# liuli33/CMLPL

Hardware: AMD Instinct MI355X
Metric: HSI patches/sec per training step (higher is better)
Workload: dtype f32 (convolutions: f32 operands as 3 exact bf16 pieces on the bf16 MFMA, 6 of 9 piece products, f32 accumulate, per-product worst case 2^-21 -- conv1's tap loops of the per-sample kernels as 2 fp16 pieces with power-of-two operand scales, 3 piece products, worst case 2^-20 / mean 2^-23, falling back; 1 GPU; B2: synthetic PaviaU-shaped patches 11x11x103, spectrum 103, 9 classes, 128 labelled + 128 unlabelled rows per GPU (batch 256), dual BaseNet2 fwd/bwd + contrastive/mutual losses + bank + Adam, epoch 1 (memory-bank smoothing active), in-kernel PCG4D noise / Philox dropout; global_batch=256, parallelism=dp1

## Files before the change

### cmlpl_amd/csrc/api.hip

```cpp
#include <hip/hip_runtime.h>
#include <stdlib.h>
#include <string.h>

#include <vector>

#include "../../include/cmlpl.h"
#include "kernels.hpp"

using namespace cmlpl;

namespace {

inline int64_t up4(int64_t v) { return (v + 3) & ~(int64_t)3; }
inline size_t up256(size_t v) { return (v + 255) & ~(size_t)255; }

struct Dims {
  int C, H, W, bands, K, HW, H2, W2, P2, H4, W4, P4, SF, F;
};

bool make_dims(const cmlpl_shape* s, Dims* d) {
  if (!s) return false;
  d->C = s->C; d->H = s->H; d->W = s->W; d->bands = s->bands; d->K = s->K;
  if (d->C < 1 || d->C > 256 || d->H < 4 || d->W < 4 || d->bands < 1 || d->K < 1 || d->K > 64) return false;
  d->HW = d->H * d->W; d->H2 = d->H / 2; d->W2 = d->W / 2; d->P2 = d->H2 * d->W2;
// ... 204 lines not shown
  x.sigma = sigma; x.nlab = b->bt; x.philox = b->noise8 == nullptr;
  x.lab0 = sh ? sh->lab0 : 0; x.unl_base = sh ? sh->bt_g + sh->unl0 : b->bt;
  x.seed = seed; x.step = step;
  return x;
}
int fwd_core(const Dims& d, const NetRoute& r, const cmlpl_layout_t& L, int nets, int n, const float* d_params, int64_t param_stride,
             const float* d_packed, const XSrc& xs, const XSrc* xspec, float* d_sn_out, const long long* d_labels, float* d_labels_f, const float* d_xn,
             const float* d_sn, const float* d_snT,
             const float* d_dropmask, float dropout_p, int train, uint64_t seed, uint64_t step,
             const cmlpl_shard* shard, float* d_logits, float* d_feat, const NetWs& w, hipStream_t st,
             float* xn_save = nullptr, int parts = 3, bool early_feat = false);
int bwd_core(const Dims& d, const NetRoute& r, const cmlpl_layout_t& L, int nets, int n, const float* d_params, int64_t param_stride,
             const float* d_packed, const XSrc& xs, const float* d_xn, const float* d_sn, const float* d_dropmask,
             float dropout_p, int train, const float* d_dlogits, const float* d_dfeat, float* d_grads,
             int64_t grad_stride, const NetWs& w, hipStream_t st, int* dyn_cursor = nullptr, cmlpl_dyn* dyn_table = nullptr,
             int parts = 3);
}

int cmlpl_basenet2_fwd(const cmlpl_shape* shape, int nets, int n, const float* d_params, int64_t param_stride,
                       const float* d_packed, const float* d_xn, const float* d_sn, const float* d_snT,
                       const float* d_dropmask, float dropout_p, int train, uint64_t seed, uint64_t step,
                       const cmlpl_shard* shard,
                       float* d_logits, float* d_feat, void* d_workspace, size_t workspace_bytes, void* stream) {
  Dims d;
  cmlpl_layout_t L;
  if (!make_dims(shape, &d) || cmlpl_layout(shape, &L)) return CMLPL_E_SHAPE;
  if (nets < 1 || nets > 2 || n < 1 || !d_params || !d_packed || !d_xn || !d_sn || !d_logits || !d_feat ||
      !d_workspace)
    return CMLPL_E_ARG;
  if (dropout_p < 0.f || dropout_p >= 1.f) return CMLPL_E_ARG;
  NetRoute r;
// ... 81 lines not shown
  if (nets < 1 || nets > 2 || n < 1 || !d_params || !d_packed || !d_xn || !d_sn || !d_dlogits || !d_grads ||
      !d_workspace)
    return CMLPL_E_ARG;
  NetRoute r;
  NetWs w;
  if (!make_route(d, nets, n, &r) || !carve_net(d, r, nets, n, (char*)d_workspace, &w)) return CMLPL_E_SHAPE;
  if (w.bytes > workspace_bytes) return CMLPL_E_WORKSPACE;
  return bwd_core(d, r, L, nets, n, d_params, param_stride, d_packed,
                  xsrc_plain(d_xn, nets, n, (long long)d.C * d.HW, 0, 0, nullptr), d_xn, d_sn, d_dropmask, dropout_p, train, d_dlogits, d_dfeat, d_grads, grad_stride, w, (hipStream_t)stream);
}

namespace {
int bwd_core(const Dims& d, const NetRoute& r, const cmlpl_layout_t& L, int nets, int n, const float* d_params, int64_t param_stride,
             const float* d_packed, const XSrc& xs, const float* d_xn, const float* d_sn, const float* d_dropmask,
             float dropout_p, int train, const float* d_dlogits, const float* d_dfeat, float* d_grads,
             int64_t grad_stride, const NetWs& w, hipStream_t st, int* dyn_cursor, cmlpl_dyn* dyn_table, int parts) {
  const float* mask = (!train || dropout_p <= 0.f) ? nullptr : (d_dropmask ? d_dropmask : w.dropgen);
  int rc;
  const bool fused_head = r.bwd == ROUTE_A;
  uint32_t* const hstat = r.stats ? w.hstat : nullptr;
  const float* d_dfeat_head = (parts == 3) ? d_dfeat : nullptr;
  GemmTN gw_cls, gw_spe;
  {
    GemmTN& g = gw_cls;
    g.bias_in = nullptr; g.bias_in_bstride = 0; g.relu = 0;
    g.A = d_dlogits; g.a_bstride = (long long)n * d.K; g.lda = d.K; g.M = d.K;
    g.B = w.catd; g.b_bstride = (long long)n * d.F; g.ldb = d.F; g.N = d.F;
    g.C = d_grads + L.param_off[8]; g.c_bstride = grad_stride; g.ldc = d.F;
    g.bias = d_grads + L.param_off[9]; g.bias_bstride = grad_stride;
    g.R = n; g.batches = nets; g.scale = 1.f;
    GemmTN& h = gw_spe;
// ... 43 lines not shown
    if ((rc = TIMED(CMLPL_K_CONV1_WGRAD, chk(launch_wgrad3_pair(nets, n, d.H, d.W, w.a0, w.dp1, w.m1, w.part1, d.H2, d.W2,
                                  w.p1, w.dp2, w.m2, w.part2, &merged, st, hstat, h2flag,
                                  L.packed_total))))) return rc;
    (void)merged;
  }
  if (!(parts & 2)) return 0;
  if (parts == 2) {
    if (!d_dfeat) return CMLPL_E_ARG;
    if ((rc = TIMED(CMLPL_K_HEAD_BWD, chk(launch_dy_fixup(nets, n, w.y, w.ynorm, d_dfeat, w.dy, st))))) return rc;
  }
  ReduceTable rt;
  rt.count = 0; rt.total_blocks = 0; rt.grad_ns = grad_stride; rt.dyn_cursor = dyn_cursor; rt.dyn_table = dyn_table;
  Wgrad3Plan wp1, wp2;
  bool wpair = false;
  if (!plan_wgrad3_both(nets, n, d.H, d.W, d.H2, d.W2, true, &wp1, &wp2, &wpair)) return CMLPL_E_SHAPE;
  reduce_table_add(rt, w.part1, wp1.G, PART3, 1, 64, d_grads + L.param_off[2], d_grads + L.param_off[3]);
  reduce_table_add(rt, w.part2, wp2.G, PART3, 1, 64, d_grads + L.param_off[4], d_grads + L.param_off[5]);
  reduce_table_add(rt, w.part0, conv0_partials(d, r, n), conv0_partial_size(d.C), 0, d.C,
                   d_grads + L.param_off[0], d_grads + L.param_off[1]);
  return TIMED(CMLPL_K_CONV1_WRED, chk(launch_reduce_gemm(nets, rt, gw_cls, gw_spe, st)));
}

int check_batch(const Dims& d, const cmlpl_batch* b) {
  if (!b || b->bt < 1 || b->btu < 1 || !b->d_xl || !b->d_xu) return CMLPL_E_ARG;
  if (b->d_cube == nullptr) return (b->d_xpl && b->d_xpu) ? 0 : CMLPL_E_ARG;
  if (b->d_xpl || b->d_xpu || !b->d_lab_pix || !b->d_unl_pix || b->cube_rows < 1 || b->cube_cols < 1) return CMLPL_E_ARG;
  if (d.H != d.W || b->cube_rows < d.H || b->cube_cols < d.W || cube_feed_lds(d.C, d.W) > LDS_MAX) return CMLPL_E_SHAPE;
  return 0;
}
}

}
namespace {
int forward_impl(const cmlpl_shape* shape, const cmlpl_hparams* hp, const cmlpl_batch* batch, const cmlpl_shard* shard,
                 const float* d_params, const float* d_packed, const float* d_dropmask, int train, uint64_t seed,
// ... 71 lines not shown
  return forward_impl(shape, hp, batch, shard, d_params, d_packed, d_dropmask, train, seed, step, d_logits, nullptr, nullptr,
                      d_workspace, workspace_bytes, stream, DynRef(), 2);
}
int cmlpl_forward(const cmlpl_shape* shape, const cmlpl_hparams* hp, const cmlpl_batch* batch, const cmlpl_shard* shard,
                  const float* d_params, const float* d_packed, const float* d_dropmask, int train, uint64_t seed,
                  uint64_t step, float* d_logits, float* d_feat, float* d_labels_f, void* d_workspace,
                  size_t workspace_bytes, void* stream) {
  return forward_impl(shape, hp, batch, shard, d_params, d_packed, d_dropmask, train, seed, step, d_logits, d_feat,
                      d_labels_f, d_workspace, workspace_bytes, stream, DynRef());
}
}
namespace {
int backward_impl(const cmlpl_shape* shape, const cmlpl_hparams* hp, const cmlpl_batch* batch, const cmlpl_shard* shard,
                  const float* d_params, const float* d_packed, const float* d_dropmask, int train, uint64_t seed,
                  uint64_t step, const float* d_dlogits, const float* d_dfeat, float* d_grads, int64_t grad_stride,
                  void* d_workspace, size_t workspace_bytes, void* stream, DynRef dyn, int* dyn_cursor, int parts = 3);
}
extern "C" {

int cmlpl_backward_data(const cmlpl_shape* shape, const cmlpl_hparams* hp, const cmlpl_batch* batch, const cmlpl_shard* shard,
                        const float* d_params, const float* d_packed, const float* d_dropmask, int train, uint64_t seed,
                        uint64_t step, const float* d_dlogits, void* d_workspace, size_t workspace_bytes, void* stream) {
  return backward_impl(shape, hp, batch, shard, d_params, d_packed, d_dropmask, train, seed, step, d_dlogits, nullptr,
                       nullptr, 0, d_workspace, workspace_bytes, stream, DynRef(), nullptr, 1);
}
int cmlpl_backward_weights(const cmlpl_shape* shape, const cmlpl_hparams* hp, const cmlpl_batch* batch,
                           const cmlpl_shard* shard, const float* d_params, const float* d_packed, const float* d_dropmask,
                           int train, uint64_t seed, uint64_t step, const float* d_dlogits, const float* d_dfeat,
                           float* d_grads, int64_t grad_stride, void* d_workspace, size_t workspace_bytes, void* stream) {
  return backward_impl(shape, hp, batch, shard, d_params, d_packed, d_dropmask, train, seed, step, d_dlogits, d_dfeat,
                       d_grads, grad_stride, d_workspace, workspace_bytes, stream, DynRef(), nullptr, 2);
}

int cmlpl_backward(const cmlpl_shape* shape, const cmlpl_hparams* hp, const cmlpl_batch* batch, const cmlpl_shard* shard,
                   const float* d_params, const float* d_packed, const float* d_dropmask, int train, uint64_t seed,
                   uint64_t step, const float* d_dlogits, const float* d_dfeat, float* d_grads, int64_t grad_stride,
                   void* d_workspace, size_t workspace_bytes, void* stream) {
  return backward_impl(shape, hp, batch, shard, d_params, d_packed, d_dropmask, train, seed, step, d_dlogits, d_dfeat,
                       d_grads, grad_stride, d_workspace, workspace_bytes, stream, DynRef(), nullptr);
}
}
namespace {
int backward_impl(const cmlpl_shape* shape, const cmlpl_hparams* hp, const cmlpl_batch* batch, const cmlpl_shard* shard,
                  const float* d_params, const float* d_packed, const float* d_dropmask, int train, uint64_t seed,
                  uint64_t step, const float* d_dlogits, const float* d_dfeat, float* d_grads, int64_t grad_stride,
                  void* d_workspace, size_t workspace_bytes, void* stream, DynRef dyn, int* dyn_cursor, int parts) {
  Dims d;
  cmlpl_layout_t L;
  if (!make_dims(shape, &d) || cmlpl_layout(shape, &L)) return CMLPL_E_SHAPE;
  if (!hp || !d_params || !d_packed || !d_dlogits || ((parts & 2) && !d_grads) || !d_workspace)
    return CMLPL_E_ARG;
  if (int brc = check_batch(d, batch)) return brc;
  const int n = batch->bt + batch->btu;
  NetRoute r;
  NetWs nw;
  if (!make_route(d, 2, n, &r) || !carve_net(d, r, 2, n, (char*)d_workspace, &nw)) return CMLPL_E_SHAPE;
  StepWs sw;
  carve_step(d, n, n, (char*)d_workspace + nw.bytes, &sw);
  if (nw.bytes + ((char*)sw.dlogits - ((char*)d_workspace + nw.bytes)) > workspace_bytes) return CMLPL_E_WORKSPACE;
  const bool copy = r.xn_copy();
  const XSrc xs = xsrc_plain(sw.xn, 2, n, (long long)d.C * d.HW, seed, step, shard, dyn);
  return bwd_core(d, r, L, 2, n, d_params, L.param_total, d_packed, xs,
                  copy ? sw.xn : nullptr, sw.sn, d_dropmask, hp->dropout_p, train, d_dlogits, d_dfeat, d_grads,
                  grad_stride, nw, (hipStream_t)stream, dyn_cursor, dyn_cursor ? (cmlpl_dyn*)dyn.table : nullptr, parts);
}
}
extern "C" {

namespace {
int fill_loss_args(const Dims& d, const cmlpl_shard* sh, const float* d_logits, const float* d_feat,
                   const int64_t* d_labels, const cmlpl_banks* banks, int smooth, float adap_mask,
                   const cmlpl_hparams* hp, void* ws, size_t ws_bytes, LossArgs* out,
                   const cmlpl_gathered* gth = nullptr, const RowSel* sel = nullptr) {
  if (!sh || !banks || !hp || !ws) return CMLPL_E_ARG;
  if (gth == nullptr && (!d_logits || !d_feat || !d_labels)) return CMLPL_E_ARG;
  if (gth != nullptr && (!gth->d_recv_feat || !gth->d_logits_local || gth->world < 1 || gth->bt_local < 1 || gth->btu_local < 1 ||
                         gth->world * gth->bt_local != sh->bt_g || gth->world * gth->btu_local != sh->btu_g ||
                         sh->nunl != gth->btu_local || sh->unl0 % gth->btu_local != 0 ||
                         (sh->nlab != 0 && (sh->nlab != gth->bt_local || sh->lab0 % gth->bt_local != 0))))
// ... 314 lines not shown
                             io->d_unl_pix};
  if ((rc = forward_impl(shape, hp, &batch, &sh, io->d_params, io->d_packed, io->d_dropmask, train, io->seed,
                         io->step, io->d_logits, io->d_feat, nullptr, io->d_workspace, io->workspace_bytes, stream, dyn, 3,
                         sym_mode)))
    return rc;
  const RowSel sel = batch_sel(&batch, dyn);
  if (cps) {
    if ((rc = cps_loss_impl(shape, io->bt, io->btu, io->d_logits, io->d_labels, hp, io->d_scalars, sw.dlogits,
                            (int64_t*)sw.probs, sw.loss,
                            loss_ws_floats(n, n, n, d.K, io->banks.Q > n ? io->banks.Q : n) * 4, stream, &sel)))
      return rc;
  } else if ((rc = loss_both(shape, io->bt, io->btu, io->d_logits, io->d_feat, io->d_labels, &io->banks,
                      io->smooth, io->adap_mask, hp, io->d_scalars, sw.dlogits, sw.dfeat, sw.probs, sw.loss,
                      loss_ws_floats(n, n, n, d.K, io->banks.Q > n ? io->banks.Q : n) * 4, stream, &sel)))
    return rc;
  if ((rc = backward_impl(shape, hp, &batch, &sh, io->d_params, io->d_packed, io->d_dropmask, train, io->seed,
                          io->step, sw.dlogits, cps ? nullptr : sw.dfeat, io->d_grads, L.param_total, io->d_workspace,
                          io->workspace_bytes, stream, dyn, io->d_dyn_cursor))) return rc;
  if (io->apply_update)
    return adam_impl(shape, 2, io->d_params, L.param_total, io->d_grads, L.param_total, io->d_m, io->d_v,
                     (dyn.table != nullptr && io->adam_t < 1) ? 1 : io->adam_t, hp, io->d_packed, stream, dyn, opt);
  if (opt != nullptr && opt->d_norms != nullptr)
    return grad_norm_impl(shape, 2, io->d_grads, L.param_total, opt->max_norm, opt->d_partials, opt->d_norms, stream, dyn);
  return 0;
}
int cmlpl_train_step(const cmlpl_shape* shape, const cmlpl_hparams* hp, const cmlpl_step_io* io, void* stream) {
  return cmlpl_train_step_opt(shape, hp, io, nullptr, stream);
}

struct StepGraph { hipGraph_t graph; hipGraphExec_t exec; };

int cmlpl_step_graph_create_opt(const cmlpl_shape* shape, const cmlpl_hparams* hp, const cmlpl_step_io* io,
                                const cmlpl_optim* opt, void* stream, void** graph_out) {
// ... 555 lines not shown
```

### cmlpl_amd/csrc/conv0.hip

```cpp
#include "common.hpp"
#include "kernels.hpp"
#include "gemm_tn.hpp"

namespace cmlpl {

constexpr int C0_KMAX = 128;

template <int KCAP>
__global__ __launch_bounds__(256) void conv0_fwd_kernel(const float* __restrict__ xn, const float* __restrict__ w0t,
                                                        long long w0t_ns, const float* __restrict__ b,
                                                        long long pstride, float* __restrict__ a0, int n, int C,
                                                        int HW) {
  extern __shared__ __attribute__((aligned(16))) float wl[];
  const int tid = threadIdx.x, lane = tid & 63, l31 = lane & 31, hh = lane >> 5;
  const int wave = __builtin_amdgcn_readfirstlane(tid >> 6);
  const int net = blockIdx.y;
  const int Cp = (C + 1) & ~1, KK = Cp >> 1;
  const long long M = (long long)n * HW;
  const long long m = ((long long)blockIdx.x * 4 + wave) * 32 + l31;
  const long long mm = (m < M) ? m : 0;
  const int sample = (int)(mm / HW), pix = (int)(mm - (long long)sample * HW);
  const float* ap = xn + ((long long)net * n + sample) * C * HW + pix;
  float av[KCAP];
#pragma unroll
// ... 341 lines not shown
  }
}

__global__ __launch_bounds__(256) void partial_reduce_kernel(ReduceTable t) {
  __shared__ __attribute__((aligned(16))) float red[16][64];
  partial_reduce_block(t, (int)blockIdx.x, (int)blockIdx.y, red);
}

__global__ __launch_bounds__(256) void reduce_gemm_kernel(ReduceTable t, int reduce_blocks, GemmTN2 g) {
  __shared__ GemmTNShared sh;
  const int bid = (int)blockIdx.x;
  if (bid < reduce_blocks) partial_reduce_block(t, bid % t.total_blocks, bid / t.total_blocks, (float (*)[64])&sh.red[0][0][0]);
  else gemm_tn_block(g, bid - reduce_blocks, sh);
}

hipError_t launch_reduce_gemm(int nets, const ReduceTable& t, const GemmTN& g0, const GemmTN& g1, hipStream_t st) {
  GemmTN2 g;
  g.p[0] = g0; g.p[1] = g1; g.nblk0 = gemm_tn_blocks(g0);
  const int rb = t.total_blocks * nets, gb = g.nblk0 + gemm_tn_blocks(g1);
  hipLaunchKernelGGL(reduce_gemm_kernel, dim3(rb + gb), dim3(256), 0, st, t, rb, g);
  return hipGetLastError();
}

void reduce_table_add(ReduceTable& t, const float* part, int G, int PS, int mode, int C, float* dW, float* db) {
  ReduceProb& p = t.p[t.count++];
  p.part = part; p.dW = dW; p.db = db; p.G = G; p.PS = PS; p.mode = mode; p.C = C; p.blk0 = t.total_blocks;
  p.el = 256;
  t.total_blocks += (PS + 255) / 256;
}

hipError_t launch_partial_reduce(int nets, const ReduceTable& t, hipStream_t st) {
  hipLaunchKernelGGL(partial_reduce_kernel, dim3(t.total_blocks, nets), dim3(256), 0, st, t);
  return hipGetLastError();
}

int conv0_partial_size(int C) { return conv0_partial_rows(C) * 64 + 64; }

int plan_conv0_wgrad_G(int n, int C, int HW) {
  (void)C; (void)HW;
  int G = n < 256 ? n : 256;
  return G < 1 ? 1 : G;
}

// ... 27 lines not shown
```

### cmlpl_amd/csrc/gemm_tn.hpp

```cpp
#pragma once
#include "common.hpp"
#include "kernels.hpp"

namespace cmlpl {

constexpr int GT_DEPTH = 16;

struct GemmTN2 { GemmTN p[2]; int nblk0; };
struct GemmTNShared { __attribute__((aligned(16))) float red[3][16][64]; float ared[4][64]; };

__device__ __forceinline__ void gemm_tn_block(const GemmTN2& t, int bid, GemmTNShared& sh) {
  const int tid = threadIdx.x, lane = tid & 63, l31 = lane & 31, hh = lane >> 5;
  const int wave = __builtin_amdgcn_readfirstlane(tid >> 6);
  const int pi = (bid >= t.nblk0) ? 1 : 0;
  const GemmTN g = t.p[pi];
  int b = bid - (pi ? t.nblk0 : 0);
  const int NTg = (g.N + 31) >> 5, MTg = (g.M + 31) >> 5;
  const int nt = b % NTg; b /= NTg;
  const int mt = b % MTg;
  const int bz = b / MTg;
  const float* A = g.A + (long long)bz * g.a_bstride;
  const float* B = g.B + (long long)bz * g.b_bstride;
  const int i = mt * 32 + l31, j = nt * 32 + l31;
  const bool iv = i < g.M, jv = j < g.N;
  const float* ap = A + (iv ? i : 0);
  const float* bp = B + (jv ? j : 0);
  const int R = g.R;
  const int pairs = (R + 1) >> 1;
  const int ppw = (pairs + 3) >> 2;
  const int t0 = wave * ppw, t1 = (t0 + ppw < pairs) ? t0 + ppw : pairs;
  f32x16 acc = zero16();
  float asum = 0.f;
  for (int tb = t0; tb < t1; tb += GT_DEPTH) {
    float av[GT_DEPTH], bv[GT_DEPTH];
    int seg = 0, off = 0;
    if (g.b_seg_rows > 0) { const int r0 = 2 * tb + hh; seg = r0 / g.b_seg_rows; off = r0 - seg * g.b_seg_rows; }
#pragma unroll
    for (int q = 0; q < GT_DEPTH; ++q) {
      const int r = 2 * (tb + q) + hh;
      const bool rv = (tb + q < t1) && (r < R);
      const int rc = rv ? r : 0;
      const long long bo = g.b_seg_rows > 0 ? (rv ? (long long)seg * g.b_seg_stride + (long long)off * g.ldb : 0)
                                            : (long long)rc * g.ldb;
      const float a = ap[(long long)rc * g.lda], b = bp[bo];
      av[q] = (rv && iv) ? a : 0.f;
      bv[q] = (rv && jv) ? b : 0.f;
      off += 2;
      while (g.b_seg_rows > 0 && off >= g.b_seg_rows) { off -= g.b_seg_rows; ++seg; }
    }
#pragma unroll
    for (int q = 0; q < GT_DEPTH; ++q) {
      asum += av[q];
      acc = mfma32(av[q], bv[q], acc);
    }
  }
  if (wave > 0) {
#pragma unroll
    for (int r = 0; r < 16; ++r) sh.red[wave - 1][r][lane] = acc[r];
  }
  sh.ared[wave][lane] = asum;
  __syncthreads();
  if (wave == 0) {
    float* C = g.C + (long long)bz * g.c_bstride;
    if (jv) {
#pragma unroll
      for (int r = 0; r < 16; ++r) {
        const int row = mt * 32 + acc_row(r, lane);
        float v = (((acc[r] + sh.red[0][r][lane]) + sh.red[1][r][lane]) + sh.red[2][r][lane]) * g.scale;
        if (g.bias_in != nullptr) v += g.bias_in[(long long)bz * g.bias_in_bstride + j];
        if (g.relu) v = relu_nan(v);
        if (row < g.M) C[(long long)row * g.ldc + j] = v;
      }
    }
    if (g.bias != nullptr && nt == 0) {
      float tot = (sh.ared[0][lane] + sh.ared[1][lane]) + (sh.ared[2][lane] + sh.ared[3][lane]);
      tot += __shfl_xor(tot, 32, 64);
// ... 9 lines not shown
```

### cmlpl_amd/csrc/kernels.hpp

```cpp
#pragma once
#include <hip/hip_runtime.h>
#include <stdint.h>
#include <stddef.h>
#include <stdlib.h>
#include <atomic>

#include "common.hpp"

namespace cmlpl {

constexpr int PACK_CONV = 9 * 64 * 64;
constexpr int PACK_B3 = PACK_CONV * 3 / 2;
constexpr int PACK_PER_NET = 4 * PACK_B3 + PACK_CONV;
__host__ __device__ inline long long pack_off_b3(int , int , int which) { return (long long)which * PACK_B3; }
__host__ __device__ inline long long pack_off_frag() { return 4LL * PACK_B3; }
__host__ __device__ inline int conv_b3_index(int tap, int k, int n, int p) {
  return ((((tap * 4 + (k >> 4)) * 3 + p) * 2 + (n >> 5)) * 64 + ((k >> 3) & 1) * 32 + (n & 31)) * 8 + (k & 7);
}
__host__ __device__ inline long long pack_off_w0t() { return PACK_PER_NET; }
__host__ __device__ inline long long pack_off_wst(int C) { return PACK_PER_NET + (long long)((C + 1) & ~1) * 64; }
__host__ __device__ inline long long pack_off_w0b3(int C, int bands) { return pack_off_wst(C) + (long long)bands * 1024; }
__host__ __device__ inline long long pack_off_w0b3_end(int C, int bands) { return pack_off_w0b3(C, bands) + (long long)((C + 15) / 16) * 1536; }
constexpr int H2_WEXP = 13;
constexpr int PACK_H2 = PACK_CONV;
// ... 101 lines not shown
hipError_t launch_wgrad3_pair(int nets, int n, int H1, int W1, const float* in1, const float* dpool1,
                              const uint8_t* mask1, float* part1, int H2, int W2, const float* in2,
                              const float* dpool2, const uint8_t* mask2, float* part2, bool* merged, hipStream_t st,
                              const uint32_t* hstat = nullptr ,
                              const uint32_t* h2flag = nullptr, long long h2flag_ns = 0);

hipError_t launch_conv0_fwd(int nets, int n, int C, int HW, const float* xn, const float* w0t, long long w0t_ns,
                            const float* b, long long pstride, float* a0, hipStream_t st);
bool conv0a_ok(int C, int HW);
hipError_t launch_conv0a_fwd(int nets, int n, int C, int HW, const XSrc& xs, const float* w0b3, long long w0b3_ns,
                             const float* b, long long pstride, float* a0, float* xn, hipStream_t st);
int plan_conv0_wgrad_G(int n, int C, int HW);
struct ReduceProb { const float* part; float* dW; float* db; int G, PS, mode, C, blk0, el; };
struct ReduceTable { ReduceProb p[3]; int count, total_blocks; long long grad_ns;
                     int* dyn_cursor; cmlpl_dyn* dyn_table;  };
void reduce_table_add(ReduceTable& t, const float* part, int G, int PS, int mode, int C, float* dW, float* db);
hipError_t launch_partial_reduce(int nets, const ReduceTable& t, hipStream_t st);
struct GemmTN;
hipError_t launch_reduce_gemm(int nets, const ReduceTable& t, const GemmTN& g0, const GemmTN& g1, hipStream_t st);
__host__ __device__ inline int conv0_partial_rows(int C) { return (C + 3) & ~3; }
int conv0_partial_size(int C);
hipError_t launch_conv0_wgrad(int nets, int n, int C, int HW, const float* xn, const float* da0, float* part,
                              hipStream_t st, const uint32_t* zstat = nullptr ,
                              const uint32_t* h2flag = nullptr, long long h2flag_ns = 0);

bool spe_fused_ok(int bands);
hipError_t launch_spe_fused(int nets, int n, int bands, const XSrc& xs, const float* w ,
                            const float* bias, long long p_ns, float* y, float* sn, const long long* labels,
                            float* labels_f, int bt, hipStream_t st);
hipError_t launch_spe_fwd(int nets, int n, int bands, const float* sn, const float* w, const float* b,
                          long long pstride, float* y, hipStream_t st, const long long* rows = nullptr,
                          long long sn_ns = -1);
hipError_t launch_feat_norm(int nets, int n, const float* y, float* ynorm, float* feat, long long feat_ns, hipStream_t st);
struct GemmTN {
// ... 24 lines not shown
  int fuse_conv0, fuse_conv0_bwd, fuse_tail, fuse_spe;
  int fuse_big;
  int conv3_nw8;
  int conv0a;
  int zero_skip;
  int bwd_pair;
  int f16x2;
  int conv3_ks;
  int ks8;
  int conv3_s, conv0_dma, conv0_ps;
  int wgrad3_u, wgrad3_cspl, wgrad3_r, wgrad3_ru, wgrad3_rg, wgrad3_pg1, wgrad3_pg2, wgrad3_b3, wgrad3_pair;
  int pair_wide, pair_nbw, pair_mb, pair16, pair_tall;
  int dfeat_lds;
  int mb_fast, unsup_onewg, unsup_3l, ntx_mfma;
  int ntx_ncw;
};
inline Switches read_switches() {
    auto env = [](const char* name, int dflt) { const char* v = getenv(name); return v ? atoi(v) : dflt; };
    Switches w;
    w.fuse_conv0 = env("CMLPL_FUSE_CONV0", 1); w.fuse_conv0_bwd = env("CMLPL_FUSE_CONV0_BWD", 1);
    w.fuse_tail = env("CMLPL_FUSE_TAIL", 1); w.fuse_spe = env("CMLPL_FUSE_SPE", 1);
    w.ks8 = env("CMLPL_KS8", -1); w.fuse_big = env("CMLPL_FUSE_BIG", 1); w.conv3_nw8 = env("CMLPL_CONV3_NW8", 1); w.conv3_ks = env("CMLPL_CONV3_KS", 1); w.conv0a = env("CMLPL_CONV0A", 1); w.f16x2 = env("CMLPL_F16X2", 1); w.bwd_pair = env("CMLPL_BWD_PAIR", 1); w.zero_skip = env("CMLPL_ZERO_SKIP", 1);
    w.conv3_s = env("CMLPL_CONV3_S", 0); w.conv0_dma = env("CMLPL_CONV0_DMA", 1); w.conv0_ps = env("CMLPL_CONV0_PS", 0);
    w.wgrad3_u = env("CMLPL_WGRAD3_U", 0); w.wgrad3_cspl = env("CMLPL_WGRAD3_CSPL", 0); w.wgrad3_r = env("CMLPL_WGRAD3_R", 1);
    w.wgrad3_ru = env("CMLPL_WGRAD3_RU", 0); w.wgrad3_rg = env("CMLPL_WGRAD3_RG", 0);
    w.wgrad3_pg1 = env("CMLPL_WGRAD3_PG1", 0); w.wgrad3_pg2 = env("CMLPL_WGRAD3_PG2", 0);
    w.wgrad3_b3 = env("CMLPL_WGRAD3_B3", 1); w.wgrad3_pair = env("CMLPL_WGRAD3_PAIR", 1);
    w.pair_wide = env("CMLPL_PAIR_WIDE", -1); w.pair_nbw = env("CMLPL_PAIR_NBW", 0); w.pair_mb = env("CMLPL_PAIR_MB", 0);
    w.pair16 = env("CMLPL_PAIR16", 1); w.pair_tall = env("CMLPL_PAIR_TALL", -1);
    w.dfeat_lds = env("CMLPL_DFEAT_LDS", -1);
    w.mb_fast = env("CMLPL_MB_FAST", 1); w.unsup_onewg = env("CMLPL_UNSUP_ONEWG", 1); w.unsup_3l = env("CMLPL_UNSUP_3L", 1);
    w.ntx_mfma = env("CMLPL_NTX_MFMA", 1); w.ntx_ncw = env("CMLPL_NTX_NCW", 0);
    return w;
}
inline Switches& switches_table() {
  static Switches sw = read_switches();
  return sw;
}
inline const Switches& switches() { return switches_table(); }

inline int device_cus() {
  static std::atomic<int> cache[64];
  int dev = 0;
  if (hipGetDevice(&dev) != hipSuccess) return 256;
  int v = cache[dev & 63].load(std::memory_order_relaxed);
  if (v == 0) {
    hipDeviceProp_t prop;
// ... 54 lines not shown
hipError_t launch_ntxent(const float* ei, const float* ej, int B, int D, float T, float* loss, float* gi, float* gj,
                         float* ws, hipStream_t st);

struct AdamOpt { const double* partials; float* norms; float max_norm, keep; };
hipError_t launch_adam(int nets, float* params, long long pstride, const float* grads, long long gstride,
                       float* m, float* v, long long live, long long t, float lr, float b1, float b2, float eps,
                       float* packed, const PackInfo& pi, hipStream_t st, DynRef dyn = DynRef(),
                       const AdamOpt* opt = nullptr);
float adam_keep(float lr, float weight_decay);
hipError_t launch_grad_norm(int nets, const float* grads, long long gstride, const long long* off, const long long* numel,
                            double* partials, hipStream_t st);
hipError_t launch_grad_norm_fin(int nets, const double* partials, float max_norm, float* norms, hipStream_t st,
                                DynRef dyn = DynRef());
size_t grad_norm_partials_bytes();
void adam_bias_scalars(float lr, float b1, float b2, long long t, float* step_size, float* bc2_sqrt);

hipError_t launch_ema(const float* src, float* ema, long long count, float alpha, float oma, hipStream_t st);

int lp_group(int K);

hipError_t launch_mb_select(const float* prob, const float* label, const float* low_mask, const float* high_mask, int N,
                            int Nl, int K, int* lists, int* counts, hipStream_t st);
hipError_t launch_mb_proto(const float* rep_t, int D, const int* lists, const int* counts, int N, int K, float* proto,
                           hipStream_t st);
hipError_t launch_mb_enqueue(const float* rep_t, int D, const int* lists, const int* counts, int N, int K, float* bank,
                             int* state, const int* caps, int cap_stride, hipStream_t st);
hipError_t launch_mb_push(const float* keys, int m, int D, float* bank_c, int* state_c, int cap, hipStream_t st);
hipError_t launch_mb_infonce(const float* rep, int D, const int* pool, const long long* anchor_draw, const float* pos,
                             long long pos_qstride, const float* bank_c, int cap, int head, const long long* neg_draw,
                             int Qn, int NN, float temp, float scale, float* lossq, float* ganchor, float* drep,
// ... 37 lines not shown
```

### cmlpl_amd/csrc/optim.hip

```cpp
#include "common.hpp"
#include "kernels.hpp"

#ifndef CMLPL_ABL
#define CMLPL_ABL 0
#endif

namespace cmlpl {

struct AdamArgs {
  float* params; long long pstride; const float* grads; long long gstride; float* m; float* v; long long live;
  float w1, b2, w2, step_size, bc2_sqrt, eps;
  float* packed; PackInfo pi;
  int nb_elem;
  DynRef dyn;
  const double* partials;
  float* norms;
  float max_norm, keep;
};

constexpr int NORM_PARTS = 64;
struct NormArgs {
  const float* grads; long long gstride;
  long long off[CMLPL_NUM_LIVE]; int numel[CMLPL_NUM_LIVE];
  double* partials;
// ... 32 lines not shown
  return c > 1.0f ? 1.0f : c;
}
__device__ __forceinline__ float* norms_row(float* norms, DynRef dyn) {
  const cmlpl_dyn* d = dyn_row(dyn, -1);
  return d != nullptr ? norms + 4 * uni32(d->hist_row) : norms;
}
__global__ __launch_bounds__(64) void grad_norm_fin_kernel(const double* partials, float max_norm, float* norms, DynRef dyn) {
  const int net = blockIdx.x;
  const float norm = (float)sqrt(norm_fold(partials, net));
  if (threadIdx.x == 0) {
    float* o = norms_row(norms, dyn);
    o[net] = norm; o[2 + net] = clip_coef(norm, max_norm);
  }
}

__device__ __forceinline__ float mul_alone(float a, float b) {
  float r = a * b;
  asm volatile("" : "+v"(r));
  return r;
}

template <bool OPT, bool CHUNK>
__device__ __forceinline__ float adam_update(float& mm, float& vv, float p, float g, const AdamArgs& a, float coef, float keep) {
  if (OPT) {
    g = mul_alone(g, coef);
    p = mul_alone(p, keep);
    mm = fmaf(a.w1, g - mm, mm);
    vv = CHUNK ? fmaf(g, a.w2 * g, vv * a.b2) : fmaf(vv, a.b2, (a.w2 * g) * g);
    const float denom = sqrtf(vv) / a.bc2_sqrt + a.eps;
    return fmaf(-a.step_size, mm / denom, p);
  }

  mm = mm + a.w1 * (g - mm);
  vv = vv * a.b2 + (a.w2 * g) * g;
  const float denom = sqrtf(vv) / a.bc2_sqrt + a.eps;
  return p - a.step_size * (mm / denom);
}
__device__ __forceinline__ void adam_dyn(AdamArgs& a) {
  const cmlpl_dyn* d = dyn_row(a.dyn, -1);
  if (d != nullptr) {
    a.step_size = __int_as_float(uni32(__float_as_int(d->adam_step_size)));
    a.bc2_sqrt = __int_as_float(uni32(__float_as_int(d->adam_bc2_sqrt)));
  }
}
__device__ __forceinline__ void adam_opt_factors(const AdamArgs& a, int net, float* coef, float* keep) {
  float k = a.keep, c = 1.f;
  const cmlpl_dyn* d = dyn_row(a.dyn, -1);
  if (d != nullptr) {
    const int bits = uni32(d->reserved);
    k = bits == 0 ? 1.f : __int_as_float(bits);
  }
  if (a.partials != nullptr) {
// ... 144 lines not shown
  a.params = params; a.pstride = pstride; a.grads = grads; a.gstride = gstride; a.m = m; a.v = v; a.live = live;
  a.w1 = (float)(1.0 - (double)b1); a.b2 = b2; a.w2 = (float)(1.0 - (double)b2); a.step_size = step_size;
  a.bc2_sqrt = bc2_sqrt; a.eps = eps; a.packed = (CMLPL_ABL == 40) ? nullptr : packed; a.pi = pi;
  a.nb_elem = (int)((n4 + 255) / 256);
  dim3 grid((unsigned)(a.nb_elem + ADAM_CHUNKS), nets);
  a.partials = nullptr; a.norms = nullptr; a.max_norm = 0.f; a.keep = 1.f;
  if (opt != nullptr) {
    a.partials = opt->partials; a.norms = opt->norms; a.max_norm = opt->max_norm; a.keep = opt->keep;
    hipLaunchKernelGGL(adam_kernel<true>, grid, dim3(256), 0, st, a);
  } else {
    hipLaunchKernelGGL(adam_kernel<false>, grid, dim3(256), 0, st, a);
  }
  return hipGetLastError();
}

float adam_keep(float lr, float weight_decay) { return (float)(1.0 - (double)lr * (double)weight_decay); }

hipError_t launch_grad_norm(int nets, const float* grads, long long gstride, const long long* off, const long long* numel,
                            double* partials, hipStream_t st) {
  NormArgs a;
  a.grads = grads; a.gstride = gstride; a.partials = partials;
  for (int t = 0; t < CMLPL_NUM_LIVE; ++t) { a.off[t] = off[t]; a.numel[t] = (int)numel[t]; }
  hipLaunchKernelGGL(grad_norm_kernel, dim3(NORM_PARTS, nets), dim3(256), 0, st, a);
  return hipGetLastError();
}
hipError_t launch_grad_norm_fin(int nets, const double* partials, float max_norm, float* norms, hipStream_t st, DynRef dyn) {
  hipLaunchKernelGGL(grad_norm_fin_kernel, dim3(nets), dim3(64), 0, st, partials, max_norm, norms, dyn);
  return hipGetLastError();
}
size_t grad_norm_partials_bytes() { return (size_t)2 * NORM_PARTS * sizeof(double); }
// ... 3 lines not shown
```

Before: 1.753 million patches/s.

## Fuse Adam update and weight repacking into the final gradient reduce/GEMM kernel

Adds a fused variant of the reduce+GEMM kernel that applies the Adam update right where each gradient element is finalized. It also rewrites the packed bf16/fp16 conv weight copies for updated conv weights and skips the separate Adam kernel launch. The aim is to remove one kernel launch and a second full pass over the gradients, params and moments. In exchange the reduce blocks now cover 512 elements instead of 256, and the code adds layout-dependent index math and a new path gated by an environment switch that defaults on.

```diff
diff --git a/cmlpl_amd/csrc/api.hip b/cmlpl_amd/csrc/api.hip
--- a/cmlpl_amd/csrc/api.hip
+++ b/cmlpl_amd/csrc/api.hip
@@ -242,7 +242,7 @@
              const float* d_packed, const XSrc& xs, const float* d_xn, const float* d_sn, const float* d_dropmask,
              float dropout_p, int train, const float* d_dlogits, const float* d_dfeat, float* d_grads,
              int64_t grad_stride, const NetWs& w, hipStream_t st, int* dyn_cursor = nullptr, cmlpl_dyn* dyn_table = nullptr,
-             int parts = 3);
+             int parts = 3, const AdamFuse* fuse = nullptr );
 }
 
 int cmlpl_basenet2_fwd(const cmlpl_shape* shape, int nets, int n, const float* d_params, int64_t param_stride,
@@ -354,7 +354,8 @@
 int bwd_core(const Dims& d, const NetRoute& r, const cmlpl_layout_t& L, int nets, int n, const float* d_params, int64_t param_stride,
              const float* d_packed, const XSrc& xs, const float* d_xn, const float* d_sn, const float* d_dropmask,
              float dropout_p, int train, const float* d_dlogits, const float* d_dfeat, float* d_grads,
-             int64_t grad_stride, const NetWs& w, hipStream_t st, int* dyn_cursor, cmlpl_dyn* dyn_table, int parts) {
+             int64_t grad_stride, const NetWs& w, hipStream_t st, int* dyn_cursor, cmlpl_dyn* dyn_table, int parts,
+             const AdamFuse* fuse) {
   const float* mask = (!train || dropout_p <= 0.f) ? nullptr : (d_dropmask ? d_dropmask : w.dropgen);
   int rc;
   const bool fused_head = r.bwd == ROUTE_A;
@@ -428,11 +429,13 @@
   Wgrad3Plan wp1, wp2;
   bool wpair = false;
   if (!plan_wgrad3_both(nets, n, d.H, d.W, d.H2, d.W2, true, &wp1, &wp2, &wpair)) return CMLPL_E_SHAPE;
-  reduce_table_add(rt, w.part1, wp1.G, PART3, 1, 64, d_grads + L.param_off[2], d_grads + L.param_off[3]);
-  reduce_table_add(rt, w.part2, wp2.G, PART3, 1, 64, d_grads + L.param_off[4], d_grads + L.param_off[5]);
+  if (fuse != nullptr && (parts != 3 || dyn_cursor != nullptr || fuse->gbase != d_grads)) return CMLPL_E_ARG;
+  const int el = fuse != nullptr ? REDUCE_FUSED_EL : 256;
+  reduce_table_add(rt, w.part1, wp1.G, PART3, 1, 64, d_grads + L.param_off[2], d_grads + L.param_off[3], el);
+  reduce_table_add(rt, w.part2, wp2.G, PART3, 1, 64, d_grads + L.param_off[4], d_grads + L.param_off[5], el);
   reduce_table_add(rt, w.part0, conv0_partials(d, r, n), conv0_partial_size(d.C), 0, d.C,
-                   d_grads + L.param_off[0], d_grads + L.param_off[1]);
-  return TIMED(CMLPL_K_CONV1_WRED, chk(launch_reduce_gemm(nets, rt, gw_cls, gw_spe, st)));
+                   d_grads + L.param_off[0], d_grads + L.param_off[1], el);
+  return TIMED(CMLPL_K_CONV1_WRED, chk(launch_reduce_gemm(nets, rt, gw_cls, gw_spe, st, fuse)));
 }
 
 int check_batch(const Dims& d, const cmlpl_batch* b) {
@@ -534,7 +537,8 @@
 int backward_impl(const cmlpl_shape* shape, const cmlpl_hparams* hp, const cmlpl_batch* batch, const cmlpl_shard* shard,
                   const float* d_params, const float* d_packed, const float* d_dropmask, int train, uint64_t seed,
                   uint64_t step, const float* d_dlogits, const float* d_dfeat, float* d_grads, int64_t grad_stride,
-                  void* d_workspace, size_t workspace_bytes, void* stream, DynRef dyn, int* dyn_cursor, int parts = 3);
+                  void* d_workspace, size_t workspace_bytes, void* stream, DynRef dyn, int* dyn_cursor, int parts = 3,
+                  const AdamFuse* fuse = nullptr);
 }
 extern "C" {
 
@@ -564,7 +568,8 @@
 int backward_impl(const cmlpl_shape* shape, const cmlpl_hparams* hp, const cmlpl_batch* batch, const cmlpl_shard* shard,
                   const float* d_params, const float* d_packed, const float* d_dropmask, int train, uint64_t seed,
                   uint64_t step, const float* d_dlogits, const float* d_dfeat, float* d_grads, int64_t grad_stride,
-                  void* d_workspace, size_t workspace_bytes, void* stream, DynRef dyn, int* dyn_cursor, int parts) {
+                  void* d_workspace, size_t workspace_bytes, void* stream, DynRef dyn, int* dyn_cursor, int parts,
+                  const AdamFuse* fuse) {
   Dims d;
   cmlpl_layout_t L;
   if (!make_dims(shape, &d) || cmlpl_layout(shape, &L)) return CMLPL_E_SHAPE;
@@ -582,7 +587,7 @@
   const XSrc xs = xsrc_plain(sw.xn, 2, n, (long long)d.C * d.HW, seed, step, shard, dyn);
   return bwd_core(d, r, L, 2, n, d_params, L.param_total, d_packed, xs,
                   copy ? sw.xn : nullptr, sw.sn, d_dropmask, hp->dropout_p, train, d_dlogits, d_dfeat, d_grads,
-                  grad_stride, nw, (hipStream_t)stream, dyn_cursor, dyn_cursor ? (cmlpl_dyn*)dyn.table : nullptr, parts);
+                  grad_stride, nw, (hipStream_t)stream, dyn_cursor, dyn_cursor ? (cmlpl_dyn*)dyn.table : nullptr, parts, fuse);
 }
 }
 extern "C" {
@@ -927,9 +932,19 @@
                       io->smooth, io->adap_mask, hp, io->d_scalars, sw.dlogits, sw.dfeat, sw.probs, sw.loss,
                       loss_ws_floats(n, n, n, d.K, io->banks.Q > n ? io->banks.Q : n) * 4, stream, &sel)))
     return rc;
+  AdamFuse fuse;
+  const bool fused = io->apply_update && io->adam_t >= 1 && dyn.table == nullptr && switches().fuse_adam != 0 &&
+                     (opt == nullptr || !optim_norm_wanted(opt));
+  if (fused) {
+    fuse.params = io->d_params; fuse.m = io->d_m; fuse.v = io->d_v; fuse.pstride = L.param_total; fuse.gbase = io->d_grads;
+    adam_fuse_scalars(fuse, hp->lr, hp->beta1, hp->beta2, hp->eps, io->adam_t);
+    fuse.keep = opt != nullptr ? adam_keep(hp->lr, opt->weight_decay) : 1.f;
+    fuse.packed = io->d_packed; fuse.pi = make_pack_info(d, L);
+  }
   if ((rc = backward_impl(shape, hp, &batch, &sh, io->d_params, io->d_packed, io->d_dropmask, train, io->seed,
                           io->step, sw.dlogits, cps ? nullptr : sw.dfeat, io->d_grads, L.param_total, io->d_workspace,
-                          io->workspace_bytes, stream, dyn, io->d_dyn_cursor))) return rc;
+                          io->workspace_bytes, stream, dyn, io->d_dyn_cursor, 3, fused ? &fuse : nullptr))) return rc;
+  if (fused) return 0;
   if (io->apply_update)
     return adam_impl(shape, 2, io->d_params, L.param_total, io->d_grads, L.param_total, io->d_m, io->d_v,
                      (dyn.table != nullptr && io->adam_t < 1) ? 1 : io->adam_t, hp, io->d_packed, stream, dyn, opt);
diff --git a/cmlpl_amd/csrc/conv0.hip b/cmlpl_amd/csrc/conv0.hip
--- a/cmlpl_amd/csrc/conv0.hip
+++ b/cmlpl_amd/csrc/conv0.hip
@@ -379,19 +379,179 @@
   else gemm_tn_block(g, bid - reduce_blocks, sh);
 }
 
-hipError_t launch_reduce_gemm(int nets, const ReduceTable& t, const GemmTN& g0, const GemmTN& g1, hipStream_t st) {
+__device__ __forceinline__ int red_swz(int col) { return col ^ (((col >> 4) & 7) << 1); }
+
+__device__ __forceinline__ void reduce_adam_block(const ReduceTable& t, int bx, int net, float* sm, const AdamFuse& f) {
+  int pi = 0;
+  if (t.count > 1 && bx >= t.p[1].blk0) pi = 1;
+  if (t.count > 2 && bx >= t.p[2].blk0) pi = 2;
+  const ReduceProb pr = t.p[pi];
+  const int tid = threadIdx.x, lane = tid & 63, el = lane, sl = tid >> 6;
+  const int G = pr.G, PS = pr.PS, body = PS - 64;
+  const int eb = (bx - pr.blk0) * REDUCE_FUSED_EL;
+  const bool conv3 = pr.mode == 1 && eb < body;
+  const long long offW = pr.dW - f.gbase, offB = pr.db - f.gbase;
+  int u[2];
+  long long po[2];
+#pragma unroll
+  for (int q = 0; q < 2; ++q) {
+    if (conv3) {
+      const int cil = lane & 7, co = (sl * 2 + q) * 8 + (lane >> 3);
+      u[q] = cil * 64 + co;
+      const int e = eb + u[q];
+      po[q] = offW + co * 576 + ((e >> 6) & 63) * 9 + (e >> 12);
+    } else {
+      u[q] = tid + 256 * q;
+      const int e = eb + u[q];
+      if (e >= PS) po[q] = -1;
+      else if (e >= body) po[q] = offB + (e - body);
+      else if (pr.mode == 1) po[q] = offW + (e & 63) * 576 + ((e >> 6) & 63) * 9 + (e >> 12);
+      else po[q] = (e >> 6) < pr.C ? offW + (long long)(e & 63) * pr.C + (e >> 6) : -1;
+    }
+  }
+  float* const pp = f.params + (long long)net * f.pstride;
+  float* const pm = f.m + (long long)net * f.pstride;
+  float* const pv = f.v + (long long)net * f.pstride;
+  float mq[2], vq[2], pq[2];
+#pragma unroll
+  for (int q = 0; q < 2; ++q) {
+    const long long o = po[q] < 0 ? 0 : po[q];
+    mq[q] = pm[o]; vq[q] = pv[o]; pq[q] = pp[o];
+  }
+  const float* p[2];
+#pragma unroll
+  for (int c = 0; c < 2; ++c) {
+    const int e0 = eb + (el + 64 * c) * 4;
+    p[c] = pr.part + (long long)net * G * PS + (e0 < PS ? e0 : 0);
+  }
+  float4 s0[2], s1[2];
+  s0[0] = s0[1] = s1[0] = s1[1] = make_float4(0.f, 0.f, 0.f, 0.f);
+  for (int g0 = sl; g0 < G; g0 += 32) {
+    float4 v[2][8];
+#pragma unroll
+    for (int c = 0; c < 2; ++c) {
+#pragma unroll
+      for (int q = 0; q < 8; ++q) {
+        const int g = g0 + 4 * q;
+        uint32_t keep = g < G ? 0xffffffffu : 0u;
+        asm volatile("" : "+v"(keep));
+        const float4 x = *(const float4*)(p[c] + (size_t)(g < G ? g : 0) * PS);
+        v[c][q] = make_float4(__uint_as_float(__float_as_uint(x.x) & keep), __uint_as_float(__float_as_uint(x.y) & keep),
+                              __uint_as_float(__float_as_uint(x.z) & keep), __uint_as_float(__float_as_uint(x.w) & keep));
+      }
+    }
+#pragma unroll
+    for (int c = 0; c < 2; ++c) {
+#define CMLPL_ADD4(F) s0[c].F += (v[c][0].F + v[c][1].F) + (v[c][2].F + v[c][3].F); s1[c].F += (v[c][4].F + v[c][5].F) + (v[c][6].F + v[c][7].F);
+      CMLPL_ADD4(x) CMLPL_ADD4(y) CMLPL_ADD4(z) CMLPL_ADD4(w)
+#undef CMLPL_ADD4
+    }
+  }
+  float4* red4 = (float4*)sm;
+#pragma unroll
+  for (int c = 0; c < 2; ++c)
+    red4[sl * 128 + red_swz(el + 64 * c)] = make_float4(s0[c].x + s1[c].x, s0[c].y + s1[c].y, s0[c].z + s1[c].z, s0[c].w + s1[c].w);
+  __syncthreads();
+  float* const wl = sm + 2048;
+  float* const gr = const_cast<float*>(f.gbase) + (long long)net * t.grad_ns;
+  float* const pkn = f.packed + (long long)net * f.pi.stride;
+#pragma unroll
+  for (int q = 0; q < 2; ++q) {
+    if (po[q] < 0) continue;
+    const int w = 4 * red_swz(u[q] >> 2) + (u[q] & 3);
+    const float sum = (sm[w] + sm[512 + w]) + (sm[1024 + w] + sm[1536 + w]);
+    gr[po[q]] = sum;
+    const float pn = conv3 ? adam_update<true, true>(mq[q], vq[q], pq[q], sum, f, 1.f, f.keep)
+                           : adam_update<true, false>(mq[q], vq[q], pq[q], sum, f, 1.f, f.keep);
+    pm[po[q]] = mq[q]; pv[po[q]] = vq[q]; pp[po[q]] = pn;
+    if (conv3) {
+      wl[(u[q] & 63) * 9 + (u[q] >> 6)] = pn;
+    } else if (pr.mode == 0 && eb + u[q] < body) {
+      const int e = eb + u[q], c = e >> 6, co = e & 63;
+      pkn[pack_off_w0t() + c * 64 + co] = pn;
+      uint32_t pcs[3];
+      b3_split(pn, pcs);
+      uint16_t* wb = (uint16_t*)(pkn + pack_off_w0b3(f.pi.C, f.pi.bands));
+#pragma unroll
+      for (int pc = 0; pc < 3; ++pc) wb[conv_b3_index(0, c, co, pc)] = (uint16_t)pcs[pc];
+    }
+  }
+  if (!conv3) return;
+  __syncthreads();
+  const int which = (offW == f.pi.off_w2) ? 2 : 0, tap = eb >> 12, ci0 = (eb >> 6) & 63;
+  static_assert(H2_WEXP == 13, "h2_split_w scales by 2^13");
+  bool bad = false;
+  if (tid < 64) {
+    const int co = tid;
+    uint4* bf = (uint4*)(pkn + pack_off_b3(f.pi.C, f.pi.bands, which));
+    uint4* hf = (uint4*)(pkn + pack_off_h2(f.pi.C, f.pi.bands, which));
+    uint32_t pc[8][3], ph[8][2];
+#pragma unroll
+    for (int j = 0; j < 8; ++j) {
+      const float w = wl[co * 9 + j];
+      b3_split(w, pc[j]);
+      bad |= h2_split_w(w, ph[j]);
+    }
+#pragma unroll
+    for (int pcs = 0; pcs < 3; ++pcs)
+      bf[conv_b3_index(tap, ci0, co, pcs) >> 3] =
+          make_uint4(pc[0][pcs] | (pc[1][pcs] << 16), pc[2][pcs] | (pc[3][pcs] << 16),
+                     pc[4][pcs] | (pc[5][pcs] << 16), pc[6][pcs] | (pc[7][pcs] << 16));
+#pragma unroll
+    for (int pcs = 0; pcs < 2; ++pcs)
+      hf[conv_h2_index(tap, ci0, co, pcs) >> 3] =
+          make_uint4(ph[0][pcs] | (ph[1][pcs] << 16), ph[2][pcs] | (ph[3][pcs] << 16),
+                     ph[4][pcs] | (ph[5][pcs] << 16), ph[6][pcs] | (ph[7][pcs] << 16));
+  } else if (tid < 64 + 128) {
+    const int it = tid - 64, co0 = (it & 15) * 4, cil = it >> 4, ci = ci0 + cil;
+    uint2* bd = (uint2*)(pkn + pack_off_b3(f.pi.C, f.pi.bands, which + 1));
+    uint2* hd = (uint2*)(pkn + pack_off_h2(f.pi.C, f.pi.bands, which + 1));
+    uint32_t pc[4][3], ph[4][2];
+#pragma unroll
+    for (int j = 0; j < 4; ++j) {
+      const float w = wl[(co0 + j) * 9 + cil];
+      b3_split(w, pc[j]);
+      bad |= h2_split_w(w, ph[j]);
+    }
+#pragma unroll
+    for (int pcs = 0; pcs < 3; ++pcs)
+      bd[conv_b3_index(8 - tap, co0, ci, pcs) >> 2] = make_uint2(pc[0][pcs] | (pc[1][pcs] << 16), pc[2][pcs] | (pc[3][pcs] << 16));
+#pragma unroll
+    for (int pcs = 0; pcs < 2; ++pcs)
+      hd[conv_h2_index(8 - tap, co0, ci, pcs) >> 2] = make_uint2(ph[0][pcs] | (ph[1][pcs] << 16), ph[2][pcs] | (ph[3][pcs] << 16));
+  }
+  if (bad) atomicOr((unsigned int*)(pkn + pack_off_h2flag(f.pi.C, f.pi.bands)), 1u);
+}
+
+__global__ __launch_bounds__(256) void reduce_gemm_adam_kernel(ReduceTable t, int reduce_blocks, GemmTN2 g, AdamFuse f) {
+  __shared__ GemmTNShared sh;
+  __shared__ float x0[16][64];
+  const int bid = (int)blockIdx.x;
+  if (bid < reduce_blocks) reduce_adam_block(t, bid % t.total_blocks, bid / t.total_blocks, &sh.red[0][0][0], f);
+  else gemm_tn_block<true>(g, bid - reduce_blocks, sh, &f, x0);
+}
+
+hipError_t launch_reduce_gemm(int nets, const ReduceTable& t, const GemmTN& g0, const GemmTN& g1, hipStream_t st,
+                              const AdamFuse* fu) {
   GemmTN2 g;
   g.p[0] = g0; g.p[1] = g1; g.nblk0 = gemm_tn_blocks(g0);
   const int rb = t.total_blocks * nets, gb = g.nblk0 + gemm_tn_blocks(g1);
-  hipLaunchKernelGGL(reduce_gemm_kernel, dim3(rb + gb), dim3(256), 0, st, t, rb, g);
+  if (fu != nullptr) {
+    if (t.dyn_cursor != nullptr) return hipErrorInvalidValue;
+    for (int i = 0; i < t.count; ++i)
+      if (t.p[i].el != REDUCE_FUSED_EL) return hipErrorInvalidValue;
+    hipLaunchKernelGGL(reduce_gemm_adam_kernel, dim3(rb + gb), dim3(256), 0, st, t, rb, g, *fu);
+  } else {
+    hipLaunchKernelGGL(reduce_gemm_kernel, dim3(rb + gb), dim3(256), 0, st, t, rb, g);
+  }
   return hipGetLastError();
 }
 
-void reduce_table_add(ReduceTable& t, const float* part, int G, int PS, int mode, int C, float* dW, float* db) {
+void reduce_table_add(ReduceTable& t, const float* part, int G, int PS, int mode, int C, float* dW, float* db, int el) {
   ReduceProb& p = t.p[t.count++];
   p.part = part; p.dW = dW; p.db = db; p.G = G; p.PS = PS; p.mode = mode; p.C = C; p.blk0 = t.total_blocks;
-  p.el = 256;
-  t.total_blocks += (PS + 255) / 256;
+  p.el = el;
+  t.total_blocks += (PS + el - 1) / el;
 }
 
 hipError_t launch_partial_reduce(int nets, const ReduceTable& t, hipStream_t st) {
diff --git a/cmlpl_amd/csrc/gemm_tn.hpp b/cmlpl_amd/csrc/gemm_tn.hpp
--- a/cmlpl_amd/csrc/gemm_tn.hpp
+++ b/cmlpl_amd/csrc/gemm_tn.hpp
@@ -9,7 +9,32 @@
 struct GemmTN2 { GemmTN p[2]; int nblk0; };
 struct GemmTNShared { __attribute__((aligned(16))) float red[3][16][64]; float ared[4][64]; };
 
-__device__ __forceinline__ void gemm_tn_block(const GemmTN2& t, int bid, GemmTNShared& sh) {
+__device__ __forceinline__ float mul_alone(float a, float b) {
+  float r = a * b;
+  asm volatile("" : "+v"(r));
+  return r;
+}
+
+template <bool OPT, bool CHUNK, class A>
+__device__ __forceinline__ float adam_update(float& mm, float& vv, float p, float g, const A& a, float coef, float keep) {
+  if (OPT) {
+    g = mul_alone(g, coef);
+    p = mul_alone(p, keep);
+    mm = fmaf(a.w1, g - mm, mm);
+    vv = CHUNK ? fmaf(g, a.w2 * g, vv * a.b2) : fmaf(vv, a.b2, (a.w2 * g) * g);
+    const float denom = sqrtf(vv) / a.bc2_sqrt + a.eps;
+    return fmaf(-a.step_size, mm / denom, p);
+  }
+
+  mm = mm + a.w1 * (g - mm);
+  vv = vv * a.b2 + (a.w2 * g) * g;
+  const float denom = sqrtf(vv) / a.bc2_sqrt + a.eps;
+  return p - a.step_size * (mm / denom);
+}
+
+template <bool UPD = false>
+__device__ __forceinline__ void gemm_tn_block(const GemmTN2& t, int bid, GemmTNShared& sh, const AdamFuse* f = nullptr,
+                                              float (*x0)[64] = nullptr) {
   const int tid = threadIdx.x, lane = tid & 63, l31 = lane & 31, hh = lane >> 5;
   const int wave = __builtin_amdgcn_readfirstlane(tid >> 6);
   const int pi = (bid >= t.nblk0) ? 1 : 0;
@@ -31,6 +56,24 @@
   const int t0 = wave * ppw, t1 = (t0 + ppw < pairs) ? t0 + ppw : pairs;
   f32x16 acc = zero16();
   float asum = 0.f;
+  float um[4], uv[4], up[4], bm = 0.f, bv2 = 0.f, bpar = 0.f, bg = 0.f;
+  long long uoff = 0, boff = 0;
+  bool bias_upd = false;
+  if (UPD) {
+    uoff = (long long)bz * f->pstride + (g.C - f->gbase);
+#pragma unroll
+    for (int rr = 0; rr < 4; ++rr) {
+      const int row = mt * 32 + acc_row(4 * wave + rr, lane);
+      const long long o = uoff + ((jv && row < g.M) ? (long long)row * g.ldc + j : 0);
+      um[rr] = f->m[o]; uv[rr] = f->v[o]; up[rr] = f->params[o];
+    }
+    bias_upd = wave == 0 && g.bias != nullptr && nt == 0 && hh == 0 && i < ((g.M + 3) & ~3);
+    if (bias_upd) {
+      boff = (long long)bz * f->pstride + (g.bias - f->gbase) + i;
+      bm = f->m[boff]; bv2 = f->v[boff]; bpar = f->params[boff];
+      if (!iv) bg = g.bias[(long long)bz * g.bias_bstride + i];
+    }
+  }
   for (int tb = t0; tb < t1; tb += GT_DEPTH) {
     float av[GT_DEPTH], bv[GT_DEPTH];
     int seg = 0, off = 0;
@@ -58,8 +101,40 @@
 #pragma unroll
     for (int r = 0; r < 16; ++r) sh.red[wave - 1][r][lane] = acc[r];
   }
+  if (UPD && wave == 0) {
+#pragma unroll
+    for (int r = 0; r < 16; ++r) x0[r][lane] = acc[r];
+  }
   sh.ared[wave][lane] = asum;
   __syncthreads();
+  if (UPD) {
+    float* C = g.C + (long long)bz * g.c_bstride;
+    if (jv) {
+#pragma unroll
+      for (int rr = 0; rr < 4; ++rr) {
+        const int r = 4 * wave + rr, row = mt * 32 + acc_row(r, lane);
+        float v = (((x0[r][lane] + sh.red[0][r][lane]) + sh.red[1][r][lane]) + sh.red[2][r][lane]) * g.scale;
+        if (g.bias_in != nullptr) v += g.bias_in[(long long)bz * g.bias_in_bstride + j];
+        if (g.relu) v = relu_nan(v);
+        if (row < g.M) {
+          const long long o = uoff + (long long)row * g.ldc + j;
+          C[(long long)row * g.ldc + j] = v;
+          const float pn = adam_update<true, false>(um[rr], uv[rr], up[rr], v, *f, 1.f, f->keep);
+          f->m[o] = um[rr]; f->v[o] = uv[rr]; f->params[o] = pn;
+        }
+      }
+    }
+    if (wave == 0 && g.bias != nullptr && nt == 0) {
+      float tot = (sh.ared[0][lane] + sh.ared[1][lane]) + (sh.ared[2][lane] + sh.ared[3][lane]);
+      tot += __shfl_xor(tot, 32, 64);
+      if (hh == 0 && iv) g.bias[(long long)bz * g.bias_bstride + i] = tot * g.scale;
+      if (bias_upd) {
+        const float pn = adam_update<true, false>(bm, bv2, bpar, iv ? tot * g.scale : bg, *f, 1.f, f->keep);
+        f->m[boff] = bm; f->v[boff] = bv2; f->params[boff] = pn;
+      }
+    }
+    return;
+  }
   if (wave == 0) {
     float* C = g.C + (long long)bz * g.c_bstride;
     if (jv) {
diff --git a/cmlpl_amd/csrc/kernels.hpp b/cmlpl_amd/csrc/kernels.hpp
--- a/cmlpl_amd/csrc/kernels.hpp
+++ b/cmlpl_amd/csrc/kernels.hpp
@@ -139,10 +139,19 @@
 struct ReduceProb { const float* part; float* dW; float* db; int G, PS, mode, C, blk0, el; };
 struct ReduceTable { ReduceProb p[3]; int count, total_blocks; long long grad_ns;
                      int* dyn_cursor; cmlpl_dyn* dyn_table;  };
-void reduce_table_add(ReduceTable& t, const float* part, int G, int PS, int mode, int C, float* dW, float* db);
+constexpr int REDUCE_FUSED_EL = 512;
+void reduce_table_add(ReduceTable& t, const float* part, int G, int PS, int mode, int C, float* dW, float* db, int el = 256);
 hipError_t launch_partial_reduce(int nets, const ReduceTable& t, hipStream_t st);
 struct GemmTN;
-hipError_t launch_reduce_gemm(int nets, const ReduceTable& t, const GemmTN& g0, const GemmTN& g1, hipStream_t st);
+struct AdamFuse {
+  float* params; float* m; float* v; long long pstride;
+  const float* gbase;
+  float w1, b2, w2, step_size, bc2_sqrt, eps;
+  float keep;
+  float* packed; PackInfo pi;
+};
+hipError_t launch_reduce_gemm(int nets, const ReduceTable& t, const GemmTN& g0, const GemmTN& g1, hipStream_t st,
+                              const AdamFuse* fu = nullptr);
 __host__ __device__ inline int conv0_partial_rows(int C) { return (C + 3) & ~3; }
 int conv0_partial_size(int C);
 hipError_t launch_conv0_wgrad(int nets, int n, int C, int HW, const float* xn, const float* da0, float* part,
@@ -197,6 +206,7 @@
   int dfeat_lds;
   int mb_fast, unsup_onewg, unsup_3l, ntx_mfma;
   int ntx_ncw;
+  int fuse_adam;
 };
 inline Switches read_switches() {
     auto env = [](const char* name, int dflt) { const char* v = getenv(name); return v ? atoi(v) : dflt; };
@@ -214,6 +224,7 @@
     w.dfeat_lds = env("CMLPL_DFEAT_LDS", -1);
     w.mb_fast = env("CMLPL_MB_FAST", 1); w.unsup_onewg = env("CMLPL_UNSUP_ONEWG", 1); w.unsup_3l = env("CMLPL_UNSUP_3L", 1);
     w.ntx_mfma = env("CMLPL_NTX_MFMA", 1); w.ntx_ncw = env("CMLPL_NTX_NCW", 0);
+    w.fuse_adam = env("CMLPL_FUSE_ADAM", 1);
     return w;
 }
 inline Switches& switches_table() {
@@ -298,6 +309,7 @@
                                 DynRef dyn = DynRef());
 size_t grad_norm_partials_bytes();
 void adam_bias_scalars(float lr, float b1, float b2, long long t, float* step_size, float* bc2_sqrt);
+void adam_fuse_scalars(AdamFuse& f, float lr, float b1, float b2, float eps, long long t);
 
 hipError_t launch_ema(const float* src, float* ema, long long count, float alpha, float oma, hipStream_t st);
 
diff --git a/cmlpl_amd/csrc/optim.hip b/cmlpl_amd/csrc/optim.hip
--- a/cmlpl_amd/csrc/optim.hip
+++ b/cmlpl_amd/csrc/optim.hip
@@ -1,5 +1,6 @@
 #include "common.hpp"
 #include "kernels.hpp"
+#include "gemm_tn.hpp"
 
 #ifndef CMLPL_ABL
 #define CMLPL_ABL 0
@@ -70,28 +71,6 @@
   }
 }
 
-__device__ __forceinline__ float mul_alone(float a, float b) {
-  float r = a * b;
-  asm volatile("" : "+v"(r));
-  return r;
-}
-
-template <bool OPT, bool CHUNK>
-__device__ __forceinline__ float adam_update(float& mm, float& vv, float p, float g, const AdamArgs& a, float coef, float keep) {
-  if (OPT) {
-    g = mul_alone(g, coef);
-    p = mul_alone(p, keep);
-    mm = fmaf(a.w1, g - mm, mm);
-    vv = CHUNK ? fmaf(g, a.w2 * g, vv * a.b2) : fmaf(vv, a.b2, (a.w2 * g) * g);
-    const float denom = sqrtf(vv) / a.bc2_sqrt + a.eps;
-    return fmaf(-a.step_size, mm / denom, p);
-  }
-
-  mm = mm + a.w1 * (g - mm);
-  vv = vv * a.b2 + (a.w2 * g) * g;
-  const float denom = sqrtf(vv) / a.bc2_sqrt + a.eps;
-  return p - a.step_size * (mm / denom);
-}
 __device__ __forceinline__ void adam_dyn(AdamArgs& a) {
   const cmlpl_dyn* d = dyn_row(a.dyn, -1);
   if (d != nullptr) {
@@ -266,6 +245,11 @@
   return hipGetLastError();
 }
 
+void adam_fuse_scalars(AdamFuse& f, float lr, float b1, float b2, float eps, long long t) {
+  adam_bias_scalars(lr, b1, b2, t, &f.step_size, &f.bc2_sqrt);
+  f.w1 = (float)(1.0 - (double)b1); f.b2 = b2; f.w2 = (float)(1.0 - (double)b2); f.eps = eps;
+}
+
 float adam_keep(float lr, float weight_decay) { return (float)(1.0 - (double)lr * (double)weight_decay); }
 
 hipError_t launch_grad_norm(int nets, const float* grads, long long gstride, const long long* off, const long long* numel,
```

New measurement: 1.777 million patches/s (median of 6 runs). +1.3%, better.
